# StefanHeng/Symbolic-Music-Generation

Hardware: AMD Instinct MI355X
Metric: train tokens/sec (TransfoXL seq2048 bf16), whole job (higher is better)
Workload: dtype bf16; 1 GPU; TransfoXL 12L/768d H12 dh64 F3072 T=2048 M=2048 V=1190 cutoffs=[] (SURVEY C3, mode R: fresh zero mems); per_gpu_batch=64, global_batch=64, seq_len=2048, mem_len=2048, parallelism=dp1

## Files before the change

include/musicxl.h:

```cpp
#ifndef MUSICXL_H
#define MUSICXL_H

#ifdef __cplusplus
extern "C" {
#endif

#define MXL_ABI_VERSION 2

int mxl_abi_version(void);
const char* mxl_error_string(int code);

#define MXL_GEMM_OUT_F32        0x01
#define MXL_GEMM_OUT_F32_ATOMIC 0x02
#define MXL_GEMM_BIAS           0x04
#define MXL_GEMM_RELU           0x08
#define MXL_GEMM_DROPOUT        0x10
#define MXL_GEMM_RELU_BWD       0x20
#define MXL_GEMM_ADD_AUX        0x40
int mxl_set_reserved_cus(int k);
int mxl_gemm_last_nt_kernel(void);

#define MXL_GEMM_SAVE_RELU_MASK 0x100
#define MXL_GEMM_RELU_BWD_BITS  0x200
size_t mxl_gemm_relu_mask_bytes(int M, int N);
// ... 37 lines not shown

int mxl_relattn_drd(const void* dg, const void* qr, float* d_rd, int B, int T, int H, int dh, int M, long long qr_bs,
                    int qr_rs, int drd_ld, const void* rd, int rd_rs, float* d_r_r_bias, float* d_r_w_bias_fix, void* stream);

int mxl_relattn_bwd_sparse_dg(const void* q, const void* k, const void* v, const void* rd, const float* r_w_bias,
                              const float* r_r_bias, const void* out, const void* dout, const float* lse, float* delta, void* dq,
                              void* dk, void* dv, void* dg, float* d_r_w_bias, int B, int T, int H, int dh, int M, int Kc,
                              long long q_bs, int q_rs, long long kv_bs, int kv_rs, int rd_rs, long long o_bs, int o_rs,
                              long long dq_bs, int dq_rs, long long dkv_bs, int dkv_rs, float scale, void* stream);
int mxl_relattn_fwd_phantom(const void* q, const void* k, const void* v, const void* rd, const float* r_w_bias,
                            const float* r_r_bias, void* out, float* lse, void* oph, float* mph, int B, int T, int H,
                            int dh, int M, int Kc, long long q_bs, int q_rs, long long kv_bs, int kv_rs, int rd_rs,
                            long long o_bs, int o_rs, float scale, void* stream);
int mxl_relattn_bwd_sparse_dg_oph(const void* q, const void* k, const void* v, const void* rd, const float* r_w_bias,
                                  const float* r_r_bias, const void* out, const void* dout, const float* lse,
                                  float* delta, void* dq, void* dk, void* dv, void* dg, float* d_r_w_bias,
                                  const void* oph, const float* mph, int B, int T, int H, int dh, int M, int Kc,
                                  long long q_bs, int q_rs, long long kv_bs, int kv_rs, int rd_rs, long long o_bs, int o_rs,
                                  long long dq_bs, int dq_rs, long long dkv_bs, int dkv_rs, float scale, void* stream);
int mxl_relattn_drd_recompute(const void* dg, const void* qr, float* d_rd, int B, int T, int H, int dh, int M, long long qr_bs,
                              int qr_rs, int drd_ld, const void* rd, int rd_rs, float* d_r_r_bias, float* d_r_w_bias_fix,
                              const float* lse, const float* delta, float scale, int Kc, void* stream);

size_t mxl_relattn_bwd_fused_ws_bytes(int B, int T, int H, int dh, int M);
int mxl_relattn_bwd_fused(const void* q, const void* k, const void* v, const void* rd, const float* r_w_bias,
                          const float* r_r_bias, const void* out, const void* dout, const float* lse, float* delta,
                          void* dq, void* dk, void* dv, float* d_rd, int drd_ld, float* d_r_w_bias, float* d_r_r_bias,
                          const void* oph, const float* mph, void* ws, int B, int T, int H, int dh, int M, int Kc,
                          long long q_bs, int q_rs, long long kv_bs, int kv_rs, int rd_rs, long long o_bs, int o_rs,
                          long long dq_bs, int dq_rs, long long dkv_bs, int dkv_rs, float scale, int defer_finish, void* stream);
int mxl_relattn_dq_finish(const void* ws, const void* oph, const float* mph, const float* lse, const float* delta, void* dq,
                          float* d_r_r_bias, int B, int T, int H, int dh, int M, int Kc, long long o_bs, int o_rs, long long dq_bs,
                          int dq_rs, float scale, void* stream);
int mxl_relattn_fwd_phantom2(const void* q, const void* k, const void* v, const void* rd, const float* r_w_bias,
                             const float* r_r_bias, void* out, float* lse, void* oph, float* mph, int oph_all, void* ph_ws, int B,
                             int T, int H, int dh, int M, int Kc, long long q_bs, int q_rs, long long kv_bs, int kv_rs, int rd_rs,
                             long long o_bs, int o_rs, float scale, void* stream);
size_t mxl_relattn_drd_phantom_ws_bytes(int B, int T, int H);
int mxl_relattn_drd_phantom_prep(const void* q, long long q_bs, int q_rs, const float* r_r_bias, const float* lse, void* ws, int B, int T,
                                 int H, int dh, float scale, void* stream);
int mxl_relattn_drd_phantom(const void* ws, const float* delta, float* d_rd, int B, int T, int H, int dh, int M, int drd_ld,
                            const void* rd, int rd_rs, int Kc, void* stream);

int mxl_sinusoid_table(void* out, int M, int d, int clamp_len, float drop_p, unsigned long long seed, unsigned site,
                       void* stream);
int mxl_embed_fwd(const void* ids, const void* E, void* out, int N, int d, int V, float scale, float drop_p,
                  unsigned long long seed, unsigned site, void* stream);
int mxl_embed_bwd(const void* ids, const void* dout, const void* dout2, float* dE, int N, int d, int V, float scale,
                  float drop_p, unsigned long long seed, unsigned site, void* stream);
int mxl_dropout_bf16(const void* x, void* y, long long n, float drop_p, unsigned long long seed, unsigned site,
                     void* stream);
int mxl_ln_residual_fwd(const void* x, const void* res, const float* gamma, const float* beta, void* y, void* z,
                        float* mean, float* rstd, int N, int d, float eps, float drop_p, unsigned long long seed,
                        unsigned site, void* stream);
int mxl_ln_residual_bwd(const void* dy, const void* dy2, const void* z, const float* mean, const float* rstd,
                        const float* gamma, void* dres, void* dx, float* dgamma, float* dbeta, int N, int d,
                        float drop_p, unsigned long long seed, unsigned site, void* stream);
int mxl_ln_residual_bwd_colsum(const void* dy, const void* dy2, const void* z, const float* mean, const float* rstd,
                               const float* gamma, void* dres, void* dx, float* dgamma, float* dbeta, float* dxsum, int N,
                               int d, float drop_p, unsigned long long seed, unsigned site, void* stream);
int mxl_ln_residual_bwd_add(const void* dy, const void* dy2, const void* z, const float* mean, const float* rstd,
                            const float* gamma, const void* dadd, void* dres, float* dgamma, float* dbeta, int N, int d,
                            void* stream);
int mxl_ln_residual_bwd_add_drop(const void* dy, const void* dy2, const void* z, const float* mean, const float* rstd,
                                 const float* gamma, const void* dadd, void* dres, void* dx, float* dxsum, float* dgamma,
                                 float* dbeta, int N, int d, float drop_p, unsigned long long seed, unsigned site, void* stream);
int mxl_add_rowbias_bf16(const void* x, long long x_bs, int x_rs, const float* bias, void* out, int B, int T, int n,
                         void* stream);
int mxl_colsum_bf16(const void* X, float* out, int M, int N, int ld, void* stream);
int mxl_dropout_colsum_bf16(const void* X, void* Y, float* out, int M, int N, float drop_p, unsigned long long seed,
                            unsigned site, void* stream);
int mxl_center_columns_bf16(const void* X, void* Y, int M, int N, void* stream);
int mxl_mem_update(const void* mem, const void* hid, void* out, int B, int M, int T, int d, void* stream);

int mxl_label_guard(void* labels_row0, int T, long long eos, void* stream);
int mxl_adaptive_nll_fwd(const float* logits, int ldl, const void* labels, float* nll, float* lse, float* acc2, int B,
                         int T, int V, int ncl, const int* cutoffs_host, void* stream);
int mxl_adaptive_nll_bwd(const float* logits, int ldl, const void* labels, const float* nll, const float* lse,
                         const float* acc2, void* dlogits, int ldd, int B, int T, int V, int ncl,
                         const int* cutoffs_host, float grad_scale, void* stream);
int mxl_adaptive_nll_bwd_split(const float* logits, int ldl, const void* labels, const float* nll, const float* lse,
                               const float* acc2, void* dlogits_hi, void* dlogits_lo, int ldd, int B, int T, int V, int ncl,
                               const int* cutoffs_host, float grad_scale, void* stream);
int mxl_adaptive_logprob(const float* logits, int ldl, float* out, int ldo, int N, int V, int ncl,
                         const int* cutoffs_host, void* stream);

int mxl_cluster_bucket(const void* labels, int B, int T, int V, int ncl, const int* cutoffs_host, int* perm, int* counts,
                       int* tgt_head, int* tgt_tail, void* stream);
int mxl_gather_rows_bf16(const void* src, int ld_src, const int* idx, void* dst, int n, int d, void* stream);
int mxl_scatter_add_rows_bf16(const void* src, const int* idx, void* dst, int ld_dst, int n, int d, void* stream);
int mxl_rows_lse_pick(const float* logits, long long ld, int ncols, int n_rows, const int* rows_idx, int row0, const int* tgt,
                      float* lse_out, float* pick_out, void* stream);
int mxl_bucket_nll_finish(const float* head_lse, const float* head_pick, const float* tail_lse, const float* tail_pick,
                          const int* tgt_head, const int* tgt_tail, float* nll, float* nll_tok, float* acc2, int B, int T,
                          void* stream);
int mxl_rows_softmax_grad(const float* logits, long long ld, int ncols, int n_rows, const int* rows_idx, int row0, const int* tgt,
                          const float* lse, const float* nll_tok, const float* acc2, float grad_scale, void* out_hi, void* out_lo,
                          int ldo, void* stream);

int mxl_sumsq_f32(const float* x, long long n, float* out_accum, void* stream);
int mxl_adamw_step(float* p, const float* g, float* m, float* v, void* w16, long long n, long long n_decay, float lr,
                   float beta1, float beta2, float eps, float weight_decay, int step, const float* sumsq,
                   float max_norm, float grad_scale, void* stream);
int mxl_cast_f32_bf16(const float* x, void* y, long long n, void* stream);
int mxl_cast_bf16_f32(const void* x, float* y, long long n, void* stream);
int mxl_transpose_bf16(const void* src, void* dst, int rows, int cols, int ld_src, int ld_dst, int batch,
                       long long src_bstride, long long dst_bstride, void* stream);

int mxl_decode_embed(const void* ids, int ld_ids, const int* t_dev, const void* E, void* out, int B, int d, int V,
                     float scale, void* stream);
int mxl_kv_append(const void* qkv, void* kcache, void* vcache, const int* t_dev, int B, int M, int d, int dh,
                  const float* r_r_bias, void* qr_out, void* stream);
int mxl_kv_fill(const void* qkv, void* kcache, void* vcache, int B, int T, int M, int d, int dh, void* stream);
int mxl_kv_zero_pad(void* qkv, const int* n_pad, int B, int T, int d, void* stream);
int mxl_decode_bd(const void* qr, const void* rd, float* bd, int B, int H, int dh, int M, int ld_qr, int ld_rd, void* stream);
int mxl_relattn_decode(const void* qkv, const void* kcache, const void* vcache, const float* bd, const float* r_w_bias,
                       void* out, const int* t_dev, int B, int H, int dh, int M, float scale, void* stream);
size_t mxl_relattn_decode_split_ws_bytes(int B, int H, int dh, int pieces);
int mxl_relattn_decode_split(const void* qkv, const void* kcache, const void* vcache, const float* bd, const float* r_w_bias,
                             void* out, const int* t_dev, int B, int H, int dh, int M, float scale, int pieces, float* ws,
                             int* arrived, void* stream);
int mxl_relattn_decode_split_live(const void* qkv, const void* kcache, const void* vcache, const float* bd, const float* r_w_bias,
                                  void* out, const int* t_dev, int B, int H, int dh, int M, float scale, int pieces, float* ws,
                                  int* arrived, const int* unfinished, void* stream);
int mxl_sample(const float* logprobs, int ldl, int V, void* ids, int ld_ids, const int* t_dev,
               unsigned long long* rng_ctr, unsigned long long seed, int B, int do_sample, int top_k, float top_p,
               float temperature, float repetition_penalty, float typical_p, float* out_probs, void* stream);
int mxl_sample_large(const float* logprobs, int ldl, int V, void* ids, int ld_ids, const int* t_dev,
                     const unsigned long long* rng_ctr, unsigned long long seed, int B, int do_sample, int top_k, float top_p,
                     float temperature, float repetition_penalty, float typical_p, float* out_probs, float* scratch,
                     void* stream);
int mxl_decode_advance(int* t_dev, unsigned long long* rng_ctr, void* stream);
int mxl_sample_step(const float* scores, int ldl, int V, void* ids, int ld_ids, int* t_dev, unsigned long long* rng_ctr,
                    unsigned long long seed, int B, int do_sample, int top_k, float top_p, float temperature,
                    float repetition_penalty, float typical_p, const void* E, void* emb_out, int d, float scale,
                    int* counter, int eos_id, int pad_id, int min_length, int* unfinished, int* alive, const void* cls,
                    const void* allow, const void* next, int C, int* gstate, const void* slots, const void* bars,
                    unsigned opens, unsigned need_free, unsigned need_full, int* gbar, int* grem, unsigned count, unsigned end,
                    int* gleft, void* stream);
int mxl_rules_mask(float* scores, int ldl, int B, int V, const int* t_dev, int eos_id, int pad_id, int min_length, int* unfinished,
                   int* alive, const void* cls, const void* allow, const void* next, int C, int* gstate, const void* slots,
                   const void* bars, unsigned opens, unsigned need_free, unsigned need_full, int* gbar, int* grem, unsigned count,
                   unsigned end, int* gleft, void* stream);
int mxl_rules_advance(void* ids, int ld_ids, const int* t_dev, int B, int V, int eos_id, int pad_id, int min_length, int* unfinished,
                      int* alive, const void* cls, const void* allow, const void* next, int C, int* gstate, const void* slots,
                      const void* bars, unsigned opens, unsigned need_free, unsigned need_full, int* gbar, int* grem, unsigned count,
                      unsigned end, int* gleft, void* stream);
int mxl_keyed_sample_step(const float* scores, int ldl, int V, void* ids, int ld_ids, int* t_dev, unsigned long long* rng_ctr,
                          unsigned long long seed, int B, int do_sample, int top_k, float top_p, float temperature,
                          float repetition_penalty, float typical_p, const void* E, void* emb_out, int d, float scale,
                          int* counter, int eos_id, int pad_id, int min_length, int* unfinished, int* alive, const void* cls,
                          const void* allow, const void* next, int C, int* gstate, const void* slots, const void* bars,
                          unsigned opens, unsigned need_free, unsigned need_full, int* gbar, int* grem, unsigned count, unsigned end,
                          int* gleft, const void* keys, const void* pcs, const void* inkey, int* gkey, float* out_probs, void* stream);
int mxl_keyed_rules_mask(float* scores, int ldl, int B, int V, const int* t_dev, int eos_id, int pad_id, int min_length,
                         int* unfinished, int* alive, const void* cls, const void* allow, const void* next, int C, int* gstate,
                         const void* slots, const void* bars, unsigned opens, unsigned need_free, unsigned need_full, int* gbar,
                         int* grem, unsigned count, unsigned end, int* gleft, const void* keys, const void* pcs, const void* inkey,
                         int* gkey, void* stream);
int mxl_keyed_rules_advance(void* ids, int ld_ids, const int* t_dev, int B, int V, int eos_id, int pad_id, int min_length,
                            int* unfinished, int* alive, const void* cls, const void* allow, const void* next, int C, int* gstate,
                            const void* slots, const void* bars, unsigned opens, unsigned need_free, unsigned need_full, int* gbar,
                            int* grem, unsigned count, unsigned end, int* gleft, const void* keys, const void* pcs, const void* inkey,
                            int* gkey, void* stream);
int mxl_guided_sample_step(const float* scores, int ldl, int V, void* ids, int ld_ids, int* t_dev, unsigned long long* rng_ctr,
                           unsigned long long seed, int B, int do_sample, int top_k, float top_p, float temperature,
// ... 139 lines not shown
```

symbolic_music_generation_amd/csrc/head.hip:

```cpp
#include "common.h"
#include "musicxl_internal.h"

namespace {

struct HeadGeom {
    int V, ncl;
    int cut[5];
};

__device__ __forceinline__ float wave_lse_range(const float* row, int lo, int hi, int lane, float extra_max,
                                                const float* extra, int n_extra) {
    constexpr int RMAX = 32;
    float m = -INFINITY;
    if (hi - lo <= 64 * RMAX) {
        float buf[RMAX];
#pragma unroll
        for (int k = 0; k < RMAX; k++) {
            const int j = lo + lane + 64 * k;
            buf[k] = (j < hi) ? row[j] : -INFINITY;
        }
#pragma unroll
        for (int k = 0; k < RMAX; k++) m = fmaxf(m, buf[k]);
        if (lane < n_extra) m = fmaxf(m, extra[lane]);
        m = wave_max(m);
        float s = 0.f;
#pragma unroll
        for (int k = 0; k < RMAX; k++) s += __expf(buf[k] - m);
        if (lane < n_extra) s += __expf(extra[lane] - m);
        s = wave_sum(s);
        return m + __logf(s);
    }
    for (int j = lo + lane; j < hi; j += 64) m = fmaxf(m, row[j]);
    if (lane < n_extra) m = fmaxf(m, extra[lane]);
    m = wave_max(m);
    float s = 0.f;
    for (int j = lo + lane; j < hi; j += 64) s += __expf(row[j] - m);
    if (lane < n_extra) s += __expf(extra[lane] - m);
    s = wave_sum(s);
    return m + __logf(s);
}

__global__ void label_guard_kernel(long long* labels, int T, long long eos) {
    __shared__ int any_valid;
    if (threadIdx.x == 0) any_valid = 0;
    __syncthreads();
    for (int t = 1 + threadIdx.x; t < T; t += blockDim.x)
        if (labels[t] != -100) any_valid = 1;
    __syncthreads();
    if (threadIdx.x == 0 && !any_valid && T > 1) labels[1] = eos;
}

constexpr int NLL_ROWS_PER_WAVE = 4;
__global__ __launch_bounds__(256) void nll_fwd_kernel(const float* logits, int ldl, const long long* labels, float* nll,
                                                      float* lse_out, float* acc, int B, int T, HeadGeom g) {
    __shared__ float part[8];
    const int lane = threadIdx.x & 63, wid = threadIdx.x >> 6;
    float tsum = 0.f, tcnt = 0.f;
    for (int rr = 0; rr < NLL_ROWS_PER_WAVE; rr++) {
        const int row = (blockIdx.x * 4 + wid) * NLL_ROWS_PER_WAVE + rr;
        if (row >= B * T) break;
        const int b = row / T, t = row % T;
        if (t == T - 1) continue;
        const long long lab = labels[(size_t)b * T + t + 1];
        float* out = nll + (size_t)b * (T - 1) + t;
        if (lab < 0 || lab >= g.V) {
            if (lane == 0) { *out = 0.f; lse_out[2 * (size_t)row] = 0.f; lse_out[2 * (size_t)row + 1] = 0.f; }
            continue;
        }
        const float* lr = logits + (size_t)row * ldl;
        const float head_lse = wave_lse_range(lr, 0, g.cut[1], lane, 0.f, lr + g.V, g.ncl);
        int ci = 0;
        for (int i = 1; i <= g.ncl; i++) if (lab >= g.cut[i]) ci = i;
        float v, tail_lse = 0.f;
        if (ci == 0) {
            v = head_lse - lr[lab];
        } else {
            tail_lse = wave_lse_range(lr, g.cut[ci], g.cut[ci + 1], lane, 0.f, nullptr, 0);
            v = (head_lse - lr[g.V + ci - 1]) + (tail_lse - lr[lab]);
        }
        if (lane == 0) {
            *out = v;
            lse_out[2 * (size_t)row] = head_lse;
            lse_out[2 * (size_t)row + 1] = tail_lse;
        }
        tsum += v;
        if (v != 0.f) tcnt += 1.f;
    }
    if (lane == 0) { part[wid] = tsum; part[4 + wid] = tcnt; }
    __syncthreads();
    if (threadIdx.x == 0) {
        atomicAdd(acc, (part[0] + part[1]) + (part[2] + part[3]));
        atomicAdd(acc + 1, (part[4] + part[5]) + (part[6] + part[7]));
    }
}

__global__ __launch_bounds__(256) void nll_bwd_kernel(const float* logits, int ldl, const long long* labels,
                                                      const float* nll, const float* lse_in, const float* acc,
                                                      bf16_t* dlogits, bf16_t* dlo, int ldd, int B, int T, HeadGeom g,
                                                      float gscale) {
    const int row = blockIdx.x * 4 + (threadIdx.x >> 6);
    if (row >= B * T) return;
    const int lane = threadIdx.x & 63;
    const int b = row / T, t = row % T;
    bf16_t* dr = dlogits + (size_t)row * ldd;
    bf16_t* dl = dlo ? dlo + (size_t)row * ldd : nullptr;
    long long lab = -100;
    float v = 0.f;
    if (t < T - 1) { lab = labels[(size_t)b * T + t + 1]; v = nll[(size_t)b * (T - 1) + t]; }
    if (lab < 0 || lab >= g.V || v == 0.f) {
        for (int j = lane; j < ldd; j += 64) {
            dr[j] = 0;
            if (dl) dl[j] = 0;
        }
        return;
    }
    const float cnt = fmaxf(acc[1], 1.f);
    const float gs = gscale / cnt;
    const float* lr = logits + (size_t)row * ldl;
    const float head_lse = lse_in[2 * (size_t)row], tail_lse = lse_in[2 * (size_t)row + 1];
    int ci = 0;
    for (int i = 1; i <= g.ncl; i++) if (lab >= g.cut[i]) ci = i;
    const int ncols = g.V + g.ncl;
    for (int j = lane; j < ldd; j += 64) {
        float d = 0.f;
        if (j < g.cut[1]) {
            d = __expf(lr[j] - head_lse) - ((ci == 0 && j == lab) ? 1.f : 0.f);
        } else if (j >= g.V && j < ncols) {
            d = __expf(lr[j] - head_lse) - ((ci > 0 && j == g.V + ci - 1) ? 1.f : 0.f);
        } else if (ci > 0 && j >= g.cut[ci] && j < g.cut[ci + 1]) {
            d = __expf(lr[j] - tail_lse) - (j == lab ? 1.f : 0.f);
        }
        const bf16_t hi = f2bf(d * gs);
        dr[j] = hi;
        if (dl) dl[j] = f2bf(d * gs - bf2f(hi));
    }
}

__global__ __launch_bounds__(256) void logprob_full_kernel(const float* logits, int ldl, float* out, int ldo, int N, HeadGeom g) {
    const int row = blockIdx.x * 4 + (threadIdx.x >> 6);
    if (row >= N) return;
    const int lane = threadIdx.x & 63;
    const float* lr = logits + (size_t)row * ldl;
    float* o = out + (size_t)row * ldo;
    const float head_lse = wave_lse_range(lr, 0, g.cut[1], lane, 0.f, lr + g.V, g.ncl);
    for (int j = lane; j < g.cut[1]; j += 64) o[j] = lr[j] - head_lse;
    for (int ci = 1; ci <= g.ncl; ci++) {
        const float tail_lse = wave_lse_range(lr, g.cut[ci], g.cut[ci + 1], lane, 0.f, nullptr, 0);
        const float base = lr[g.V + ci - 1] - head_lse;
        for (int j = g.cut[ci] + lane; j < g.cut[ci + 1]; j += 64) o[j] = base + (lr[j] - tail_lse);
    }
}

int make_geom(HeadGeom& g, int V, int ncl, const int* cutoffs) {
    if (V <= 0 || ncl < 0 || ncl > 3) return MXL_EINVAL;
    if (ncl > 0 && !cutoffs) return MXL_EINVAL;
    g.V = V; g.ncl = ncl; g.cut[0] = 0;
    for (int i = 0; i < ncl; i++) {
        g.cut[i + 1] = cutoffs[i];
        if (cutoffs[i] <= g.cut[i] || cutoffs[i] >= V) return MXL_EINVAL;
    }
    g.cut[ncl + 1] = V;
    for (int i = ncl + 2; i < 5; i++) g.cut[i] = V;
    return MXL_OK;
}

}

extern "C" int mxl_label_guard(void* labels_row0, int T, long long eos, void* stream) {
    MXL_CHECK_ARG(labels_row0 && T > 0);
    hipLaunchKernelGGL(label_guard_kernel, dim3(1), dim3(256), 0, (hipStream_t)stream, (long long*)labels_row0, T, eos);
    MXL_LAUNCH_CHECK();
    return MXL_OK;
}

extern "C" int mxl_adaptive_nll_fwd(const float* logits, int ldl, const void* labels, float* nll, float* lse,
                                    float* acc2, int B, int T, int V, int ncl, const int* cutoffs_host, void* stream) {
    MXL_CHECK_ARG(logits && labels && nll && lse && acc2 && B > 0 && T > 1);
    HeadGeom g;
    int rc = make_geom(g, V, ncl, cutoffs_host);
    if (rc) return rc;
    MXL_CHECK_ARG(ldl >= V + ncl);
    hipLaunchKernelGGL(nll_fwd_kernel, dim3((B * T + 4 * NLL_ROWS_PER_WAVE - 1) / (4 * NLL_ROWS_PER_WAVE)), dim3(256), 0, (hipStream_t)stream, logits, ldl,
                       (const long long*)labels, nll, lse, acc2, B, T, g);
    MXL_LAUNCH_CHECK();
    return MXL_OK;
}

extern "C" int mxl_adaptive_nll_bwd(const float* logits, int ldl, const void* labels, const float* nll, const float* lse,
                                    const float* acc2, void* dlogits, int ldd, int B, int T, int V, int ncl,
                                    const int* cutoffs_host, float grad_scale, void* stream) {
    MXL_CHECK_ARG(logits && labels && nll && lse && acc2 && dlogits && B > 0 && T > 1);
    HeadGeom g;
    int rc = make_geom(g, V, ncl, cutoffs_host);
    if (rc) return rc;
    MXL_CHECK_ARG(ldl >= V + ncl && ldd >= V + ncl);
    hipLaunchKernelGGL(nll_bwd_kernel, dim3((B * T + 3) / 4), dim3(256), 0, (hipStream_t)stream, logits, ldl,
                       (const long long*)labels, nll, lse, acc2, (bf16_t*)dlogits, (bf16_t*)nullptr, ldd, B, T, g, grad_scale);
    MXL_LAUNCH_CHECK();
    return MXL_OK;
}

extern "C" int mxl_adaptive_nll_bwd_split(const float* logits, int ldl, const void* labels, const float* nll, const float* lse,
                                          const float* acc2, void* dlogits_hi, void* dlogits_lo, int ldd, int B, int T, int V,
                                          int ncl, const int* cutoffs_host, float grad_scale, void* stream) {
    MXL_CHECK_ARG(logits && labels && nll && lse && acc2 && dlogits_hi && dlogits_lo && B > 0 && T > 1);
    HeadGeom g;
    int rc = make_geom(g, V, ncl, cutoffs_host);
    if (rc) return rc;
    MXL_CHECK_ARG(ldl >= V + ncl && ldd >= V + ncl);
    hipLaunchKernelGGL(nll_bwd_kernel, dim3((B * T + 3) / 4), dim3(256), 0, (hipStream_t)stream, logits, ldl,
                       (const long long*)labels, nll, lse, acc2, (bf16_t*)dlogits_hi, (bf16_t*)dlogits_lo, ldd, B, T, g,
                       grad_scale);
    MXL_LAUNCH_CHECK();
    return MXL_OK;
}

extern "C" int mxl_adaptive_logprob(const float* logits, int ldl, float* out, int ldo, int N, int V, int ncl,
                                    const int* cutoffs_host, void* stream) {
    MXL_CHECK_ARG(logits && out && N > 0);
    HeadGeom g;
    int rc = make_geom(g, V, ncl, cutoffs_host);
    if (rc) return rc;
    MXL_CHECK_ARG(ldl >= V + ncl && ldo >= V);
    hipLaunchKernelGGL(logprob_full_kernel, dim3((N + 3) / 4), dim3(256), 0, (hipStream_t)stream, logits, ldl, out, ldo,
                       N, g);
    MXL_LAUNCH_CHECK();
    return MXL_OK;
}
```

symbolic_music_generation_amd/ops.py:

```python
import ctypes as C
import math
import os
from typing import Optional, Sequence

import torch

from ._lib import lib, check, MusicXLError

GEMM_OUT_F32 = 0x01
GEMM_OUT_F32_ATOMIC = 0x02
GEMM_BIAS = 0x04
GEMM_RELU = 0x08
GEMM_DROPOUT = 0x10
GEMM_RELU_BWD = 0x20
GEMM_ADD_AUX = 0x40
GEMM_SAVE_RELU_MASK = 0x100
GEMM_RELU_BWD_BITS = 0x200


def mix_seed(base_seed: int, step: int) -> int:
    import torch.distributed as dist
    rank = dist.get_rank() if (dist.is_available() and dist.is_initialized()) else 0
    x = (base_seed * 0x9E3779B97F4A7C15 + rank * 0xD1B54A32D192ED03 + step * 0x2545F4914F6CDD1D) & 0xFFFFFFFFFFFFFFFF
    x ^= x >> 32
# ... 492 lines not shown
    if dxsum is not None:
        colsum(dx, dxsum, N, d)


def ln_bwd_add(dy, dy2, z, mean, rstd, gamma, dadd, dres, dgamma, dbeta):
    d = z.shape[-1]
    N = z.numel() // d
    check(lib().mxl_ln_residual_bwd_add(_p(dy), _p(dy2), _p(z), _p(mean), _p(rstd), _p(gamma), _p(dadd), _p(dres), _p(dgamma),
                                        _p(dbeta), N, d, _stream()), 'mxl_ln_residual_bwd_add')


def ln_bwd_add_drop(dy, dy2, z, mean, rstd, gamma, dadd, dres, dx, dxsum, dgamma, dbeta, p: float, seed: int, site: int):
    d = z.shape[-1]
    N = z.numel() // d
    check(lib().mxl_ln_residual_bwd_add_drop(_p(dy), _p(dy2), _p(z), _p(mean), _p(rstd), _p(gamma), _p(dadd), _p(dres), _p(dx),
                                             _p(dxsum), _p(dgamma), _p(dbeta), N, d, float(p), seed, site, _stream()),
          'mxl_ln_residual_bwd_add_drop')


def dropout_colsum(x: torch.Tensor, y: torch.Tensor, out: torch.Tensor, M: int, N: int, p: float, seed: int, site: int):
    check(lib().mxl_dropout_colsum_bf16(_p(x), _p(y), _p(out), M, N, float(p), seed, site, _stream()), 'mxl_dropout_colsum_bf16')


def colsum(x: torch.Tensor, out: torch.Tensor, M: int, N: int, ld: Optional[int] = None):
    check(lib().mxl_colsum_bf16(_p(x), _p(out), M, N, ld if ld is not None else x.stride(-2), _stream()), 'mxl_colsum_bf16')
    return out


def mem_update(mem, hid, out):
    B, M, d = mem.shape
    T = hid.shape[1]
    check(lib().mxl_mem_update(_p(mem), _p(hid), _p(out), B, M, T, d, _stream()), 'mxl_mem_update')
    return out


def phantom_sum_applies(*, T, dh, M, Kc) -> bool:
    return (dh == 64 and T % 32 == 0 and M % 256 == 0 and Kc < M + T and os.environ.get('MXL_NO_DQ8') != '1'
            and os.environ.get('MXL_DG_RECOMPUTE', '1') != '0' and os.environ.get('MXL_NO_OPH') != '1')


def set_reserved_cus(k: int) -> None:
    check(lib().mxl_set_reserved_cus(int(k)), 'mxl_set_reserved_cus')


def fused_bwd_applies(*, T, dh, M, Kc, B=None, H=None) -> bool:
    ok = (dh == 64 and T % 32 == 0 and M % 32 == 0 and M <= 8192 and Kc % 32 == 0 and (T - Kc) % 64 == 0
          and os.environ.get('MXL_NO_FUSED_BWD') != '1')
    if ok and B is not None and H is not None and Kc < M + T:
        ok = H * (T // 32) * 4352 < 2 ** 31 and B * H * T * 4 < 2 ** 31
    return ok


def relattn_fwd(q, k, v, rd, r_w_bias, r_r_bias, out, lse, *, B, T, H, dh, M, Kc, q_bs, q_rs, kv_bs, kv_rs, rd_rs,
                o_bs, o_rs, scale=None, oph=None, mph=None, oph_all=False, ph_buf=None):
    scale = scale if scale is not None else 1.0 / math.sqrt(dh)
    if oph is not None and oph_all:
        check(lib().mxl_relattn_fwd_phantom2(_p(q), _p(k), _p(v), _p(rd), _p(r_w_bias), _p(r_r_bias), _p(out), _p(lse), _p(oph),
                                             _p(mph), 1, _p(ph_buf), B, T, H, dh, M, Kc, q_bs, q_rs, kv_bs, kv_rs, rd_rs, o_bs, o_rs,
                                             float(scale), _stream()), 'mxl_relattn_fwd_phantom2')
        return out
    if oph is not None:
        check(lib().mxl_relattn_fwd_phantom(_p(q), _p(k), _p(v), _p(rd), _p(r_w_bias), _p(r_r_bias), _p(out), _p(lse), _p(oph),
                                            _p(mph), B, T, H, dh, M, Kc, q_bs, q_rs, kv_bs, kv_rs, rd_rs, o_bs, o_rs, float(scale),
                                            _stream()), 'mxl_relattn_fwd_phantom')
        return out
    check(lib().mxl_relattn_fwd(_p(q), _p(k), _p(v), _p(rd), _p(r_w_bias), _p(r_r_bias), _p(out), _p(lse), B, T, H, dh,
                                M, Kc, q_bs, q_rs, kv_bs, kv_rs, rd_rs, o_bs, o_rs, float(scale), _stream()),
          'mxl_relattn_fwd')
    return out


def label_guard(labels: torch.Tensor, eos: int):
    _req(labels, torch.int64, 'labels')
    check(lib().mxl_label_guard(_p(labels), labels.shape[1], int(eos), _stream()), 'mxl_label_guard')


def adaptive_nll_fwd(logits, labels, nll, lse, acc2, B, T, V, cutoffs=()):
    n, arr = _cut(cutoffs)
    check(lib().mxl_adaptive_nll_fwd(_p(logits), logits.stride(0), _p(labels), _p(nll), _p(lse), _p(acc2), B, T, V, n,
                                     C.cast(arr, C.c_void_p) if arr is not None else None, _stream()),
          'mxl_adaptive_nll_fwd')


def adaptive_nll_bwd(logits, labels, nll, lse, acc2, dlogits, B, T, V, cutoffs=(), grad_scale=1.0, dlogits_lo=None):
    n, arr = _cut(cutoffs)
    if dlogits_lo is not None:
        assert dlogits_lo.shape == dlogits.shape and dlogits_lo.stride(0) == dlogits.stride(0)
        check(lib().mxl_adaptive_nll_bwd_split(_p(logits), logits.stride(0), _p(labels), _p(nll), _p(lse), _p(acc2), _p(dlogits),
                                               _p(dlogits_lo), dlogits.stride(0), B, T, V, n,
                                               C.cast(arr, C.c_void_p) if arr is not None else None, float(grad_scale),
                                               _stream()), 'mxl_adaptive_nll_bwd_split')
        return
    check(lib().mxl_adaptive_nll_bwd(_p(logits), logits.stride(0), _p(labels), _p(nll), _p(lse), _p(acc2), _p(dlogits),
                                     dlogits.stride(0), B, T, V, n,
                                     C.cast(arr, C.c_void_p) if arr is not None else None, float(grad_scale), _stream()),
          'mxl_adaptive_nll_bwd')


def adaptive_logprob(logits, out, N, V, cutoffs=()):
    n, arr = _cut(cutoffs)
    check(lib().mxl_adaptive_logprob(_p(logits), logits.stride(0), _p(out), out.stride(0), N, V, n,
                                     C.cast(arr, C.c_void_p) if arr is not None else None, _stream()),
          'mxl_adaptive_logprob')
    return out


def cluster_bucket(labels, V, cutoffs, perm, counts, tgt_head, tgt_tail):
    B, T = labels.shape
    n, arr = _cut(cutoffs)
    check(lib().mxl_cluster_bucket(_p(labels), B, T, V, n, C.cast(arr, C.c_void_p), _p(perm), _p(counts), _p(tgt_head),
                                   _p(tgt_tail), _stream()), 'mxl_cluster_bucket')


def gather_rows(src, idx, dst, n):
    check(lib().mxl_gather_rows_bf16(_p(src), src.stride(-2), _p(idx), _p(dst), n, src.shape[-1], _stream()), 'mxl_gather_rows_bf16')
    return dst


def scatter_add_rows(src, idx, dst, n):
    check(lib().mxl_scatter_add_rows_bf16(_p(src), _p(idx), _p(dst), dst.stride(-2), n, src.shape[-1], _stream()),
          'mxl_scatter_add_rows_bf16')


def rows_lse_pick(logits, ncols, n_rows, tgt, lse_out, pick_out, rows_idx=None, row0=0):
    check(lib().mxl_rows_lse_pick(_p(logits), logits.stride(0), ncols, n_rows, _p(rows_idx), row0, _p(tgt), _p(lse_out),
                                  _p(pick_out), _stream()), 'mxl_rows_lse_pick')


def bucket_nll_finish(hlse, hpick, tlse, tpick, tgt_head, tgt_tail, nll, nll_tok, acc2, B, T):
    check(lib().mxl_bucket_nll_finish(_p(hlse), _p(hpick), _p(tlse), _p(tpick), _p(tgt_head), _p(tgt_tail), _p(nll), _p(nll_tok),
                                      _p(acc2), B, T, _stream()), 'mxl_bucket_nll_finish')


def rows_softmax_grad(logits, ncols, n_rows, tgt, lse, nll_tok, acc2, grad_scale, out_hi, out_lo=None, rows_idx=None, row0=0):
    check(lib().mxl_rows_softmax_grad(_p(logits), logits.stride(0), ncols, n_rows, _p(rows_idx), row0, _p(tgt), _p(lse), _p(nll_tok),
                                      _p(acc2), float(grad_scale), _p(out_hi), _p(out_lo), out_hi.stride(0), _stream()),
          'mxl_rows_softmax_grad')


def sumsq(x: torch.Tensor, out_accum: torch.Tensor):
    check(lib().mxl_sumsq_f32(_p(x), x.numel(), _p(out_accum), _stream()), 'mxl_sumsq_f32')


def adamw_step(p, g, m, v, w16, n_decay, lr, beta1, beta2, eps, weight_decay, step, sumsq_buf=None, max_norm=0.0,
               grad_scale=1.0):
    check(lib().mxl_adamw_step(_p(p), _p(g), _p(m), _p(v), _p(w16), p.numel(), n_decay, float(lr), float(beta1),
                               float(beta2), float(eps), float(weight_decay), int(step), _p(sumsq_buf), float(max_norm),
                               float(grad_scale), _stream()), 'mxl_adamw_step')


def cast_bf16(x: torch.Tensor, y: torch.Tensor):
    check(lib().mxl_cast_f32_bf16(_p(x), _p(y), x.numel(), _stream()), 'mxl_cast_f32_bf16')
    return y


def cast_f32(x: torch.Tensor, y: torch.Tensor):
    _req(x, torch.bfloat16, 'x'); _req(y, torch.float32, 'y')
    check(lib().mxl_cast_bf16_f32(_p(x), _p(y), x.numel(), _stream()), 'mxl_cast_bf16_f32')
    return y


def center_columns(x: torch.Tensor, y: torch.Tensor):
    M, N = x.shape
    check(lib().mxl_center_columns_bf16(_p(x), _p(y), M, N, _stream()), 'mxl_center_columns_bf16')
    return y


def transpose(src: torch.Tensor, dst: torch.Tensor, rows: int, cols: int, *, ld_src=None, ld_dst=None, batch=1,
# ... 401 lines not shown
```

symbolic_music_generation_amd/xl_engine.py:

```python
import math
import os
from collections import OrderedDict
from typing import Dict, List, Optional, Sequence, Tuple

import torch

from . import ops
from ._lib import MusicXLError

F = ops


def _r8(n: int) -> int:
    return (n + 7) // 8 * 8


class ParamLayout:

    def __init__(self, cfg):
        d, Fi, H, dh, V, L = cfg.d_model, cfg.d_inner, cfg.n_head, cfg.d_head, cfg.vocab_size, cfg.n_layer
        ncl = len(cfg.cutoffs)
        self.n_head_rows = V + ncl
        self.head_rows_padded = _r8(V + ncl)
        decay: List[Tuple[str, Tuple[int, ...]]] = [('transformer.word_emb.emb_layers.0.weight', (V, d))]
# ... 422 lines not shown
        for r0 in range(0, N, ch):
            n = min(ch, N - r0)
            x = hid[r0:r0 + n]
            ops.gemm(x, hb.wp, hl, n, c1 + ncl, d, flags=F.GEMM_OUT_F32 | F.GEMM_BIAS, bias=hb.bp)
            ops.rows_softmax_grad(hl, c1 + ncl, n, hb.tgt_head, hb.hlse, hb.nll_tok, ws.acc, grad_scale, dl, dl_lo, row0=r0)
            for term in (dl_lo, dl):
                ops.colsum(term, G[boff:boff + c1], n, c1)
                ops.colsum(term[:, c1:], G[boff + V:boff + V + ncl], n, ncl, ld=hb.ldh)
                ops.gemm(term, x, g_head_w[:c1], c1, d, n, trans_a=True, trans_b=True, flags=AT, ksplits=self._ks(c1, d, n))
                ops.gemm(term[:, c1:], x, g_head_w[V:V + ncl], ncl, d, n, trans_a=True, trans_b=True, flags=AT, lda=hb.ldh,
                         ksplits=self._ks(ncl, d, n))
            ops.gemm(dl_lo, hb.wp, dy[r0:r0 + n], n, d, hb.ldh, trans_b=True)
            ops.gemm(dl, hb.wp, dy[r0:r0 + n], n, d, hb.ldh, trans_b=True, flags=F.GEMM_ADD_AUX, aux=dy[r0:r0 + n])
        del hl, dl, dl_lo
        bounds = (0,) + cut + (V,)
        for i in range(1, ncl + 1):
            n_i, lo, S = hb.counts_host[i], bounds[i], bounds[i + 1] - bounds[i]
            if n_i == 0:
                continue
            ldt = _r8(S)
            ch = self._chunk_rows(n_i, ldt)
            tl = torch.empty(ch, ldt, device=self.dev, dtype=torch.float32)
            dtl = torch.empty(ch, ldt, device=self.dev, dtype=torch.bfloat16)
            hc = torch.empty(ch, d, device=self.dev, dtype=torch.bfloat16)
            dhc = torch.empty(ch, d, device=self.dev, dtype=torch.bfloat16)
            for j0 in range(0, n_i, ch):
                n = min(ch, n_i - j0)
                idx = hb.perm[i, j0:j0 + n]
                ops.gather_rows(hid, idx, hc, n)
                ops.gemm(hc, head_w[lo:lo + S], tl, n, S, d, flags=F.GEMM_OUT_F32 | F.GEMM_BIAS, bias=self.P[boff + lo:boff + lo + S])
                ops.rows_softmax_grad(tl, S, n, hb.tgt_tail, hb.tlse, hb.nll_tok, ws.acc, grad_scale, dtl, None, rows_idx=idx)
                ops.colsum(dtl, G[boff + lo:boff + lo + S], n, S)
                ops.gemm(dtl, hc, g_head_w[lo:lo + S], S, d, n, trans_a=True, trans_b=True, flags=AT, ksplits=self._ks(S, d, n))
                ops.gemm(dtl, head_w[lo:lo + ldt], dhc, n, d, ldt, trans_b=True)
                ops.scatter_add_rows(dhc, idx, dy, n)
            del tl, dtl, hc, dhc

    def _chunked_logprobs(self, hid, N, head_w, head_b):
        c = self.cfg
        V, cut, d = c.vocab_size, tuple(c.cutoffs), c.d_model
        nrow, nrow_p = self.layout.n_head_rows, self.layout.head_rows_padded
        lp = torch.empty(N, V, device=self.dev, dtype=torch.float32)
        ch = self._chunk_rows(N, nrow_p)
        lg = torch.empty(ch, nrow_p, device=self.dev, dtype=torch.float32)
        for r0 in range(0, N, ch):
            n = min(ch, N - r0)
            ops.gemm(hid[r0:r0 + n], head_w, lg, n, nrow, d, flags=F.GEMM_OUT_F32 | F.GEMM_BIAS, bias=head_b)
            ops.adaptive_logprob(lg, lp[r0:r0 + n], n, V, cut)
        return lp

    def zero_grad(self):
        if self.G is None:
            self.G = torch.zeros_like(self.P)
        else:
            self.G.zero_()

    @staticmethod
    def _ks(m, n, k=0):
        tiles = ((m + 127) // 128) * ((n + 127) // 128)
        if k >= 49152:
            return 12 if tiles <= 48 else max(1, min(24, 1440 // tiles))
        return max(1, min(24, 512 // max(tiles, 1)))

    def backward(self, grad_scale: float = 1.0, layer_done=None):
        ws, c = self._last, self.cfg
        B, T, Kc, p, seed = ws.B, ws.T, ws.Kc, ws.p, ws.seed
        d, H, dh, L, M, Fi = c.d_model, c.n_head, c.d_head, c.n_layer, c.mem_len, c.d_inner
        V, cut = c.vocab_size, tuple(c.cutoffs)
        if self.WT is None:
            self._refresh_wt(allocate=True)
        N = B * T
        G = self.G
        nrow, nrow_p = self.layout.n_head_rows, self.layout.head_rows_padded
        AT = F.GEMM_OUT_F32_ATOMIC
        dscale = 1.0 / (1.0 - p) if p > 0 else 1.0

        def gw(l, suffix):
            return self._lw(l, suffix, G)

        dy, dy2 = ws.dA, None
        if self.bucketed_head:
            self._bucketed_head_bwd(ws, dy, B, T, grad_scale)
        else:
            ops.adaptive_nll_bwd(ws.logits, ws.labels, ws.nll, ws.hlse, ws.acc, ws.dlogits, B, T, V, cut, grad_scale,
                                 dlogits_lo=ws.dlogits_lo)
            head_w = self.W[:nrow_p * d].view(nrow_p, d)
            g_head_w = G[:nrow_p * d].view(nrow_p, d)
            boff = self.layout.entries['crit.out_layers.0.bias'][0]
            for term in (ws.dlogits_lo, ws.dlogits):
                ops.colsum(term, G[boff:boff + nrow], N, nrow)
                ops.gemm(term, ws.hid, g_head_w, nrow_p, d, N, trans_a=True, trans_b=True, flags=AT,
                         ksplits=self._ks(nrow_p, d, N))
            ops.gemm(ws.dlogits_lo, self.WT['head'], dy, N, d, self._head_kp())
            ops.gemm(ws.dlogits, self.WT['head'], dy, N, d, self._head_kp(), flags=F.GEMM_ADD_AUX, aux=dy)
        if p > 0:
            ops.dropout(dy, dy, p, seed=seed, site=self.SITE_FINAL)
        st = dict(B=B, T=T, H=H, dh=dh, M=M, Kc=Kc, q_bs=Kc * 3 * d, q_rs=3 * d, kv_bs=Kc * 3 * d, kv_rs=3 * d, rd_rs=d,
                  o_bs=T * d, o_rs=d)
        ops.center_columns(ws.phi, ws.phi_c)
        for l in reversed(range(L)):
            h_in = ws.h[l]
            ops.ln_residual_bwd(dy, dy2, ws.z2[l], ws.st2[l][0], ws.st2[l][1], self._lw(l, 'pos_ff.layer_norm.weight', self.P),
                                ws.dC, ws.dD, gw(l, 'pos_ff.layer_norm.weight'), gw(l, 'pos_ff.layer_norm.bias'),
                                drop_p=p, seed=seed, site=self._site(l, 2), dxsum=gw(l, 'pos_ff.CoreNet.3.bias'))
            ops.gemm(ws.dD, ws.a[l], gw(l, 'pos_ff.CoreNet.3.weight'), d, Fi, N, trans_a=True, trans_b=True, flags=AT,
                     ksplits=self._ks(d, Fi, N))
            if ws.rmask is not None:
                ops.gemm(ws.dD, self._lwt(l, 'pos_ff.CoreNet.3.weight'), ws.dF, N, Fi, d, flags=F.GEMM_RELU_BWD_BITS,
                         aux=ws.rmask[l], alpha=dscale, colsum=gw(l, 'pos_ff.CoreNet.0.bias'))
            else:
                ops.gemm(ws.dD, self._lwt(l, 'pos_ff.CoreNet.3.weight'), ws.dF, N, Fi, d, flags=F.GEMM_RELU_BWD,
                         aux=ws.a[l], alpha=dscale, colsum=gw(l, 'pos_ff.CoreNet.0.bias'))
            ops.gemm(ws.dF, ws.h1[l], gw(l, 'pos_ff.CoreNet.0.weight'), Fi, d, N, trans_a=True, trans_b=True, flags=AT,
                     ksplits=self._ks(Fi, d, N))
            ops.gemm(ws.dF, self._lwt(l, 'pos_ff.CoreNet.0.weight'), ws.dD, N, d, Fi)
            ops.ln_residual_bwd(ws.dC, ws.dD, ws.z1[l], ws.st1[l][0], ws.st1[l][1],
                                self._lw(l, 'dec_attn.layer_norm.weight', self.P), ws.dA, ws.dB,
                                gw(l, 'dec_attn.layer_norm.weight'), gw(l, 'dec_attn.layer_norm.bias'), drop_p=p,
                                seed=seed, site=self._site(l, 0))
            ops.gemm(ws.dB, ws.av[l], gw(l, 'dec_attn.o_net.weight'), d, d, N, trans_a=True, trans_b=True, flags=AT,
                     ksplits=self._ks(d, d, N))
            delta_ready = False
            if ws.fused_bwd and not os.environ.get('MXL_HEADDOT_OFF'):
                delta_ready = ops.gemm_headdot(ws.dB, self._lwt(l, 'dec_attn.o_net.weight'), ws.dC, N, d, d, ws.av[l], T, ws.delta)
            else:
                ops.gemm(ws.dB, self._lwt(l, 'dec_attn.o_net.weight'), ws.dC, N, d, d)
            qkv, dqkv = ws.qkv[l], ws.dqkv
            ws.d_rd.zero_()
            if ws.fused_bwd:
                ops.relattn_bwd_fused(qkv[:, Kc - T:, :d], qkv[:, :, d:2 * d], qkv[:, :, 2 * d:], ws.rd[l],
                                      self._lw(l, 'dec_attn.r_w_bias', self.P), self._lw(l, 'dec_attn.r_r_bias', self.P), ws.av[l],
                                      ws.dC, ws.lse[l], ws.delta, dqkv[:, Kc - T:, :d], dqkv[:, :, d:2 * d], dqkv[:, :, 2 * d:],
                                      ws.d_rd, gw(l, 'dec_attn.r_w_bias'), gw(l, 'dec_attn.r_r_bias'), ws.dq_slabs, ws.qr,
                                      dq_bs=Kc * 3 * d, dq_rs=3 * d, dkv_bs=Kc * 3 * d, dkv_rs=3 * d,
                                      oph=ws.oph[l].view(B, T, d) if ws.oph is not None else None,
                                      mph=ws.mph[l] if ws.oph is not None else None,
                                      ph_buf=ws.ph[l] if ws.ph is not None else None, ph_ready=ws.ph is not None,
                                      delta_ready=delta_ready, **st)
            else:
                ops.relattn_bwd(qkv[:, Kc - T:, :d], qkv[:, :, d:2 * d], qkv[:, :, 2 * d:], ws.rd[l],
                                self._lw(l, 'dec_attn.r_w_bias', self.P), self._lw(l, 'dec_attn.r_r_bias', self.P), ws.av[l],
                                ws.dC, ws.lse[l], ws.delta, dqkv[:, Kc - T:, :d], dqkv[:, :, d:2 * d], dqkv[:, :, 2 * d:],
                                ws.dg, gw(l, 'dec_attn.r_w_bias'), gw(l, 'dec_attn.r_r_bias'), dq_bs=Kc * 3 * d, dq_rs=3 * d,
                                dkv_bs=Kc * 3 * d, dkv_rs=3 * d, d_rd=ws.d_rd, qr_buf=ws.qr,
                                oph=ws.oph[l].view(B, T, d) if ws.oph is not None else None,
                                mph=ws.mph[l] if ws.oph is not None else None, **st)
            ops.cast_bf16(ws.d_rd, ws.d_rd16)
            ops.gemm(ws.d_rd16, ws.phi_c, gw(l, 'dec_attn.r_net.weight'), d, d, M, trans_a=True, trans_b=True, flags=AT,
                     ksplits=self._ks(d, d))
            if ws.has_mem:
                dqkv[:, :M, :d].zero_()
                x_qkv = ws.cat[l].view(B * Kc, d)
            else:
                x_qkv = h_in
            ops.gemm(dqkv.view(B * Kc, 3 * d), x_qkv, gw(l, 'dec_attn.qkv_net.weight'), 3 * d, d, B * Kc, trans_a=True,
                     trans_b=True, flags=AT, ksplits=self._ks(3 * d, d, B * Kc))
            if ws.has_mem:
                ops.gemm_batched(dqkv[:, M:], self._lw(l, 'dec_attn.qkv_net.weight'), ws.dB, T, d, 3 * d, lda=3 * d,
                                 ldb=d, ldc=d, trans_b=True, batch=B, bdiv=1, sA=(Kc * 3 * d, 0), sB=(0, 0), sC=(T * d, 0))
            else:
                ops.gemm(dqkv.view(N, 3 * d), self._lwt(l, 'dec_attn.qkv_net.weight'), ws.dB, N, d, 3 * d)
            dy, dy2 = ws.dA, ws.dB
            if layer_done is not None:
                layer_done(l)
        E_g = self.layout.view(G, 'transformer.word_emb.emb_layers.0.weight')
        ops.embed_bwd(ws.ids, dy, E_g, math.sqrt(d), drop_p=p, seed=seed, site=self.SITE_EMB, dout2=dy2)

    def optimizer_step(self, lr: float, betas=(0.9, 0.999), eps=1e-8, weight_decay=0.01, max_grad_norm=1.0,
                       grad_scale: float = 1.0):
        if self.m is None:
            self.m = torch.zeros_like(self.P)
            self.v = torch.zeros_like(self.P)
        self.step_count += 1
# ... 12 lines not shown
```

Before: 852,400 tokens/s.

## Fuse head bias gradient column-sum into vectorized NLL backward kernel

Rewrites the adaptive NLL backward kernel so each block handles 64 rows with 4-wide vector loads and stores, and optionally accumulates the bias-gradient column sums in registers, reducing them through shared memory and atomics. The engine now passes the bias gradient slice into this kernel and drops the two separate colsum launches over the hi and lo dlogits. This removes two extra full reads of the bf16 logit-gradient buffers and improves memory coalescing. The cost is more atomic traffic per block and higher register pressure from the per-lane column accumulators.

```diff
diff --git a/include/musicxl.h b/include/musicxl.h
--- a/include/musicxl.h
+++ b/include/musicxl.h
@@ -143,6 +143,9 @@
 int mxl_adaptive_nll_bwd_split(const float* logits, int ldl, const void* labels, const float* nll, const float* lse,
                                const float* acc2, void* dlogits_hi, void* dlogits_lo, int ldd, int B, int T, int V, int ncl,
                                const int* cutoffs_host, float grad_scale, void* stream);
+int mxl_adaptive_nll_bwd_bias(const float* logits, int ldl, const void* labels, const float* nll, const float* lse,
+                              const float* acc2, void* dlogits_hi, void* dlogits_lo, int ldd, int B, int T, int V, int ncl,
+                              const int* cutoffs_host, float grad_scale, float* dbias, void* stream);
 int mxl_adaptive_logprob(const float* logits, int ldl, float* out, int ldo, int N, int V, int ncl,
                          const int* cutoffs_host, void* stream);
 
diff --git a/symbolic_music_generation_amd/csrc/head.hip b/symbolic_music_generation_amd/csrc/head.hip
--- a/symbolic_music_generation_amd/csrc/head.hip
+++ b/symbolic_music_generation_amd/csrc/head.hip
@@ -94,45 +94,114 @@
     }
 }
 
+constexpr int NLLB_ROWS = 64;
+__device__ __forceinline__ void nll_split(float d, float gs, bool want_lo, bf16_t& hi, bf16_t& lo) {
+#pragma clang fp contract(off)
+    const float pg = d * gs;
+    hi = f2bf(pg);
+    lo = want_lo ? f2bf(pg - bf2f(hi)) : (bf16_t)0;
+}
+__device__ __forceinline__ float nll_grad(const HeadGeom& g, int j, float x, int ci, long long lab, float head_lse, float tail_lse) {
+    float d = 0.f;
+    if (j < g.cut[1]) {
+        d = __expf(x - head_lse) - ((ci == 0 && j == lab) ? 1.f : 0.f);
+    } else if (j >= g.V && j < g.V + g.ncl) {
+        d = __expf(x - head_lse) - ((ci > 0 && j == g.V + ci - 1) ? 1.f : 0.f);
+    } else if (ci > 0 && j >= g.cut[ci] && j < g.cut[ci + 1]) {
+        d = __expf(x - tail_lse) - (j == lab ? 1.f : 0.f);
+    }
+    return d;
+}
+
+template <int NQ, bool CS>
 __global__ __launch_bounds__(256) void nll_bwd_kernel(const float* logits, int ldl, const long long* labels,
                                                       const float* nll, const float* lse_in, const float* acc,
                                                       bf16_t* dlogits, bf16_t* dlo, int ldd, int B, int T, HeadGeom g,
-                                                      float gscale) {
-    const int row = blockIdx.x * 4 + (threadIdx.x >> 6);
-    if (row >= B * T) return;
-    const int lane = threadIdx.x & 63;
-    const int b = row / T, t = row % T;
-    bf16_t* dr = dlogits + (size_t)row * ldd;
-    bf16_t* dl = dlo ? dlo + (size_t)row * ldd : nullptr;
-    long long lab = -100;
-    float v = 0.f;
-    if (t < T - 1) { lab = labels[(size_t)b * T + t + 1]; v = nll[(size_t)b * (T - 1) + t]; }
-    if (lab < 0 || lab >= g.V || v == 0.f) {
-        for (int j = lane; j < ldd; j += 64) {
-            dr[j] = 0;
-            if (dl) dl[j] = 0;
-        }
-        return;
-    }
-    const float cnt = fmaxf(acc[1], 1.f);
-    const float gs = gscale / cnt;
-    const float* lr = logits + (size_t)row * ldl;
-    const float head_lse = lse_in[2 * (size_t)row], tail_lse = lse_in[2 * (size_t)row + 1];
-    int ci = 0;
-    for (int i = 1; i <= g.ncl; i++) if (lab >= g.cut[i]) ci = i;
-    const int ncols = g.V + g.ncl;
-    for (int j = lane; j < ldd; j += 64) {
-        float d = 0.f;
-        if (j < g.cut[1]) {
-            d = __expf(lr[j] - head_lse) - ((ci == 0 && j == lab) ? 1.f : 0.f);
-        } else if (j >= g.V && j < ncols) {
-            d = __expf(lr[j] - head_lse) - ((ci > 0 && j == g.V + ci - 1) ? 1.f : 0.f);
-        } else if (ci > 0 && j >= g.cut[ci] && j < g.cut[ci + 1]) {
-            d = __expf(lr[j] - tail_lse) - (j == lab ? 1.f : 0.f);
-        }
-        const bf16_t hi = f2bf(d * gs);
-        dr[j] = hi;
-        if (dl) dl[j] = f2bf(d * gs - bf2f(hi));
+                                                      float gscale, float* dbias) {
+    extern __shared__ __attribute__((aligned(16))) char nllb_smem[];
+    const int lane = threadIdx.x & 63, wid = threadIdx.x >> 6;
+    const int nq = ldd >> 2;
+    float cs[NQ > 0 ? NQ : 1][4];
+#pragma unroll
+    for (int q = 0; q < (NQ > 0 ? NQ : 1); q++)
+#pragma unroll
+        for (int e = 0; e < 4; e++) cs[q][e] = 0.f;
+    for (int rr = 0; rr < NLLB_ROWS / 4; rr++) {
+        const int row = blockIdx.x * NLLB_ROWS + rr * 4 + wid;
+        if (row >= B * T) break;
+        const int b = row / T, t = row % T;
+        bf16_t* dr = dlogits + (size_t)row * ldd;
+        bf16_t* dl = dlo ? dlo + (size_t)row * ldd : nullptr;
+        long long lab = -100;
+        float v = 0.f;
+        if (t < T - 1) { lab = labels[(size_t)b * T + t + 1]; v = nll[(size_t)b * (T - 1) + t]; }
+        if (lab < 0 || lab >= g.V || v == 0.f) {
+            if (NQ > 0) {
+#pragma unroll
+                for (int q = 0; q < NQ; q++) {
+                    const int c = lane + 64 * q;
+                    if (c < nq) {
+                        *reinterpret_cast<u32x2*>(dr + 4 * c) = u32x2{0u, 0u};
+                        if (dl) *reinterpret_cast<u32x2*>(dl + 4 * c) = u32x2{0u, 0u};
+                    }
+                }
+            } else {
+                for (int j = lane; j < ldd; j += 64) {
+                    dr[j] = 0;
+                    if (dl) dl[j] = 0;
+                }
+            }
+            continue;
+        }
+        const float cnt = fmaxf(acc[1], 1.f);
+        const float gs = gscale / cnt;
+        const float* lr = logits + (size_t)row * ldl;
+        const float head_lse = lse_in[2 * (size_t)row], tail_lse = lse_in[2 * (size_t)row + 1];
+        int ci = 0;
+        for (int i = 1; i <= g.ncl; i++) if (lab >= g.cut[i]) ci = i;
+        if (NQ > 0) {
+            f32x4 x[NQ > 0 ? NQ : 1];
+#pragma unroll
+            for (int q = 0; q < NQ; q++) {
+                const int c = lane + 64 * q;
+                x[q] = f32x4{0.f, 0.f, 0.f, 0.f};
+                if (4 * c < ldl && c < nq) x[q] = *reinterpret_cast<const f32x4*>(lr + 4 * c);
+            }
+#pragma unroll
+            for (int q = 0; q < NQ; q++) {
+                const int c = lane + 64 * q;
+                if (c < nq) {
+                    bf16_t hi[4], lo[4];
+#pragma unroll
+                    for (int e = 0; e < 4; e++) {
+                        const float d = nll_grad(g, 4 * c + e, x[q][e], ci, lab, head_lse, tail_lse);
+                        nll_split(d, gs, dl != nullptr, hi[e], lo[e]);
+                        if (CS) cs[q][e] += bf2f(hi[e]) + bf2f(lo[e]);
+                    }
+                    *reinterpret_cast<u32x2*>(dr + 4 * c) = (u32x2{(uint32_t)hi[0] | ((uint32_t)hi[1] << 16), (uint32_t)hi[2] | ((uint32_t)hi[3] << 16)});
+                    if (dl) *reinterpret_cast<u32x2*>(dl + 4 * c) = (u32x2{(uint32_t)lo[0] | ((uint32_t)lo[1] << 16), (uint32_t)lo[2] | ((uint32_t)lo[3] << 16)});
+                }
+            }
+        } else {
+            for (int j = lane; j < ldd; j += 64) {
+                const float d = nll_grad(g, j, j < g.V + g.ncl ? lr[j] : 0.f, ci, lab, head_lse, tail_lse);
+                bf16_t hi, lo;
+                nll_split(d, gs, dl != nullptr, hi, lo);
+                dr[j] = hi;
+                if (dl) dl[j] = lo;
+            }
+        }
+    }
+    if (CS && NQ > 0) {
+        float* red = reinterpret_cast<float*>(nllb_smem);
+#pragma unroll
+        for (int q = 0; q < NQ; q++) {
+            const int c = lane + 64 * q;
+            if (c < nq) *reinterpret_cast<f32x4*>(red + (size_t)wid * ldd + 4 * c) = f32x4{cs[q][0], cs[q][1], cs[q][2], cs[q][3]};
+        }
+        __syncthreads();
+        for (int j = threadIdx.x; j < g.V + g.ncl; j += 256)
+            atomicAdd(dbias + j, (red[j] + red[ldd + j]) + (red[2 * ldd + j] + red[3 * ldd + j]));
     }
 }
 
@@ -186,33 +255,55 @@
     return MXL_OK;
 }
 
-extern "C" int mxl_adaptive_nll_bwd(const float* logits, int ldl, const void* labels, const float* nll, const float* lse,
-                                    const float* acc2, void* dlogits, int ldd, int B, int T, int V, int ncl,
-                                    const int* cutoffs_host, float grad_scale, void* stream) {
-    MXL_CHECK_ARG(logits && labels && nll && lse && acc2 && dlogits && B > 0 && T > 1);
+static int nll_bwd_launch(const float* logits, int ldl, const void* labels, const float* nll, const float* lse, const float* acc2,
+                          void* dhi, void* dlo, int ldd, int B, int T, int V, int ncl, const int* cutoffs_host, float grad_scale,
+                          float* dbias, void* stream) {
+    MXL_CHECK_ARG(logits && labels && nll && lse && acc2 && dhi && B > 0 && T > 1);
     HeadGeom g;
     int rc = make_geom(g, V, ncl, cutoffs_host);
     if (rc) return rc;
     MXL_CHECK_ARG(ldl >= V + ncl && ldd >= V + ncl);
-    hipLaunchKernelGGL(nll_bwd_kernel, dim3((B * T + 3) / 4), dim3(256), 0, (hipStream_t)stream, logits, ldl,
-                       (const long long*)labels, nll, lse, acc2, (bf16_t*)dlogits, (bf16_t*)nullptr, ldd, B, T, g, grad_scale);
+    hipStream_t s = (hipStream_t)stream;
+    const int N = B * T;
+    const bool vec = (ldl % 4) == 0 && (ldd % 4) == 0 && ldd <= 256 * 8 && ((uintptr_t)logits % 16) == 0 && ((uintptr_t)dhi % 8) == 0 &&
+                     (!dlo || ((uintptr_t)dlo % 8) == 0);
+    const dim3 grid((N + NLLB_ROWS - 1) / NLLB_ROWS);
+    const size_t smem = dbias && vec ? (size_t)4 * ldd * sizeof(float) : 0;
+#define NLLB_LAUNCH(NQ, CS)                                                                                                      \
+    hipLaunchKernelGGL((nll_bwd_kernel<NQ, CS>), grid, dim3(256), smem, s, logits, ldl, (const long long*)labels, nll, lse, acc2, \
+                       (bf16_t*)dhi, (bf16_t*)dlo, ldd, B, T, g, grad_scale, dbias)
+    if (!vec) NLLB_LAUNCH(0, false);
+    else if (ldd <= 256 * 5) { if (dbias) NLLB_LAUNCH(5, true); else NLLB_LAUNCH(5, false); }
+    else { if (dbias) NLLB_LAUNCH(8, true); else NLLB_LAUNCH(8, false); }
+#undef NLLB_LAUNCH
     MXL_LAUNCH_CHECK();
-    return MXL_OK;
+    if (dbias && !vec) {
+        if (dlo && (rc = mxl_colsum_bf16(dlo, dbias, N, V + ncl, ldd, stream))) return rc;
+        return mxl_colsum_bf16(dhi, dbias, N, V + ncl, ldd, stream);
+    }
+    return MXL_OK;
+}
+
+extern "C" int mxl_adaptive_nll_bwd(const float* logits, int ldl, const void* labels, const float* nll, const float* lse,
+                                    const float* acc2, void* dlogits, int ldd, int B, int T, int V, int ncl,
+                                    const int* cutoffs_host, float grad_scale, void* stream) {
+    return nll_bwd_launch(logits, ldl, labels, nll, lse, acc2, dlogits, nullptr, ldd, B, T, V, ncl, cutoffs_host, grad_scale, nullptr, stream);
 }
 
 extern "C" int mxl_adaptive_nll_bwd_split(const float* logits, int ldl, const void* labels, const float* nll, const float* lse,
                                           const float* acc2, void* dlogits_hi, void* dlogits_lo, int ldd, int B, int T, int V,
                                           int ncl, const int* cutoffs_host, float grad_scale, void* stream) {
-    MXL_CHECK_ARG(logits && labels && nll && lse && acc2 && dlogits_hi && dlogits_lo && B > 0 && T > 1);
-    HeadGeom g;
-    int rc = make_geom(g, V, ncl, cutoffs_host);
-    if (rc) return rc;
-    MXL_CHECK_ARG(ldl >= V + ncl && ldd >= V + ncl);
-    hipLaunchKernelGGL(nll_bwd_kernel, dim3((B * T + 3) / 4), dim3(256), 0, (hipStream_t)stream, logits, ldl,
-                       (const long long*)labels, nll, lse, acc2, (bf16_t*)dlogits_hi, (bf16_t*)dlogits_lo, ldd, B, T, g,
-                       grad_scale);
-    MXL_LAUNCH_CHECK();
-    return MXL_OK;
+    MXL_CHECK_ARG(dlogits_lo);
+    return nll_bwd_launch(logits, ldl, labels, nll, lse, acc2, dlogits_hi, dlogits_lo, ldd, B, T, V, ncl, cutoffs_host, grad_scale, nullptr,
+                          stream);
+}
+
+extern "C" int mxl_adaptive_nll_bwd_bias(const float* logits, int ldl, const void* labels, const float* nll, const float* lse,
+                                         const float* acc2, void* dlogits_hi, void* dlogits_lo, int ldd, int B, int T, int V, int ncl,
+                                         const int* cutoffs_host, float grad_scale, float* dbias, void* stream) {
+    MXL_CHECK_ARG(dbias);
+    return nll_bwd_launch(logits, ldl, labels, nll, lse, acc2, dlogits_hi, dlogits_lo, ldd, B, T, V, ncl, cutoffs_host, grad_scale, dbias,
+                          stream);
 }
 
 extern "C" int mxl_adaptive_logprob(const float* logits, int ldl, float* out, int ldo, int N, int V, int ncl,
diff --git a/symbolic_music_generation_amd/ops.py b/symbolic_music_generation_amd/ops.py
--- a/symbolic_music_generation_amd/ops.py
+++ b/symbolic_music_generation_amd/ops.py
@@ -598,8 +598,15 @@
           'mxl_adaptive_nll_fwd')
 
 
-def adaptive_nll_bwd(logits, labels, nll, lse, acc2, dlogits, B, T, V, cutoffs=(), grad_scale=1.0, dlogits_lo=None):
+def adaptive_nll_bwd(logits, labels, nll, lse, acc2, dlogits, B, T, V, cutoffs=(), grad_scale=1.0, dlogits_lo=None, dbias=None):
     n, arr = _cut(cutoffs)
+    if dbias is not None:
+        assert dlogits_lo is None or (dlogits_lo.shape == dlogits.shape and dlogits_lo.stride(0) == dlogits.stride(0))
+        check(lib().mxl_adaptive_nll_bwd_bias(_p(logits), logits.stride(0), _p(labels), _p(nll), _p(lse), _p(acc2), _p(dlogits),
+                                              _p(dlogits_lo), dlogits.stride(0), B, T, V, n,
+                                              C.cast(arr, C.c_void_p) if arr is not None else None, float(grad_scale), _p(dbias),
+                                              _stream()), 'mxl_adaptive_nll_bwd_bias')
+        return
     if dlogits_lo is not None:
         assert dlogits_lo.shape == dlogits.shape and dlogits_lo.stride(0) == dlogits.stride(0)
         check(lib().mxl_adaptive_nll_bwd_split(_p(logits), logits.stride(0), _p(labels), _p(nll), _p(lse), _p(acc2), _p(dlogits),
diff --git a/symbolic_music_generation_amd/xl_engine.py b/symbolic_music_generation_amd/xl_engine.py
--- a/symbolic_music_generation_amd/xl_engine.py
+++ b/symbolic_music_generation_amd/xl_engine.py
@@ -528,13 +528,12 @@
         if self.bucketed_head:
             self._bucketed_head_bwd(ws, dy, B, T, grad_scale)
         else:
+            boff = self.layout.entries['crit.out_layers.0.bias'][0]
             ops.adaptive_nll_bwd(ws.logits, ws.labels, ws.nll, ws.hlse, ws.acc, ws.dlogits, B, T, V, cut, grad_scale,
-                                 dlogits_lo=ws.dlogits_lo)
+                                 dlogits_lo=ws.dlogits_lo, dbias=G[boff:boff + nrow])
             head_w = self.W[:nrow_p * d].view(nrow_p, d)
             g_head_w = G[:nrow_p * d].view(nrow_p, d)
-            boff = self.layout.entries['crit.out_layers.0.bias'][0]
             for term in (ws.dlogits_lo, ws.dlogits):
-                ops.colsum(term, G[boff:boff + nrow], N, nrow)
                 ops.gemm(term, ws.hid, g_head_w, nrow_p, d, N, trans_a=True, trans_b=True, flags=AT,
                          ksplits=self._ks(nrow_p, d, N))
             ops.gemm(ws.dlogits_lo, self.WT['head'], dy, N, d, self._head_kp())
```

Measured after the change: 869,300 tokens/s (median of 4 runs). +2.0%, better.
